# zgcr/SimpleAICV_pytorch_training_examples

Hardware: AMD Instinct MI355X
Metric: training images/sec/node (higher is better)
Workload: dtype bf16; 1 GPU; resnet50 3x224x224 synthetic training step (fwd+loss+bwd+all-reduce+optimizer), per-GPU batch 256; model=resnet50, global_batch=256, per_gpu_batch=256, parallelism=dp1, step_graph=True, bn_statistics=fixed-order partial rows, deterministic=True, loop=tools.scripts.train_classification, optimizer=SGD, param_groups=2

## Files before the change

simpleaicv_pytorch_training_examples_amd/csrc/igemm.hip:

```cpp
#include <type_traits>

#include <stdlib.h>
#include "common.h"
#include "saicv_internal.h"
#include "det.h"
#include "../../include/saicv_hip.h"

namespace {

struct FastDiv {
    uint32_t mul, s1, s2;
};
DEVINL uint32_t fdiv(uint32_t n, FastDiv d) {
    const uint32_t t = __umulhi(d.mul, n);
    return (t + ((n - t) >> d.s1)) >> d.s2;
}

constexpr int nt_stages(int bm, int bn) { return (bm == 256 && bn == 128) ? 3 : 4; }
constexpr int nt_stages_kc8(int bm, int bn) { return (bm + bn) * 128 * 3 <= 150 * 1024 ? 3 : 2; }

struct NTParams {
    const void* src;
    const void* wgt;
    void* out;
// ... 752 lines not shown
    if (bstats) {
        __syncthreads();
        float* red = reinterpret_cast<float*>(smem);
        const bool have = ncol + OEPC <= p.Nn;
#pragma unroll
        for (int j = 0; j < OEPC; ++j) {
            const float mu = have ? p.bs_mean[ncol + j] : 0.f, is = have ? p.bs_invstd[ncol + j] : 0.f;
            red[(orow0 * 2 + 0) * BN_T + oc * OEPC + j] = bag[j];
            red[(orow0 * 2 + 1) * BN_T + oc * OEPC + j] = is * fmaf(-mu, bag[j], bax[j]);
        }
        __syncthreads();
        const size_t prow = (size_t)((MODE == 1 && cs > 1) ? blockIdx.y : 0) * p.bs_rows + tile_m;
        for (int c = tid; c < 2 * BN_T; c += NTHREADS) {
            const int which = c / BN_T, col = c - which * BN_T;
            float a = 0.f;
            for (int r = 0; r < RPP; ++r) a += red[(r * 2 + which) * BN_T + col];
            const int n = tile_n * BN_T + col;
            if (n < p.Nn) {
                float* dst = (which ? p.bs_gx : p.bs_g) + (p.stat_atomic_rows ? prow % p.stat_atomic_rows : prow) * (size_t)p.Nn + n;
                if (p.stat_atomic_rows) unsafeAtomicAdd(dst, a); else *dst = a;
            }
        }
    }
    }
#ifdef SAICV_NT_TIMELINE
    if (tl_on && tix == (int)blockIdx.x) {
        NT_STAMP(6);
        asm volatile("s_waitcnt vmcnt(0)" ::: "memory");
        NT_STAMP(7);
        if (tid == 0) {
            unsigned long long* rec = p.timeline + ((size_t)blockIdx.y * gridDim.x + blockIdx.x) * 16;
            unsigned int hw, xcc;
            asm volatile("s_getreg_b32 %0, hwreg(HW_REG_HW_ID)" : "=s"(hw));
            asm volatile("s_getreg_b32 %0, hwreg(HW_REG_XCC_ID)" : "=s"(xcc));
#pragma unroll
            for (int i = 0; i < 8; ++i) rec[i] = tl_t[i];
            rec[8] = ((unsigned long long)xcc << 32) | hw;
            rec[9] = __builtin_amdgcn_s_memrealtime();
            rec[10] = tl_rt0;
            rec[11] = tl_t[8]; rec[12] = tl_t[9]; rec[13] = tl_t[10];
        }
    }
#endif
    }
}


struct TNParams {
    const void* dy;
    const void* src;
    float* dw;
    float* dbias;
    uint32_t dy_bytes, src_bytes;
    int H, W, C;
    int OH, OW;
    int R, S, stride, pad;
    int M, Cout, Kd;
    int tiles_a, tiles_b;
    int m_per_split;
    int d_img, d_oh, d_ow;
    FastDiv fd_ohw, fd_ow;
    saicv::DetSink det;
};

template <typename T, int BA, int BB, int NWA, int NWB>
__global__ __launch_bounds__(64 * NWA * NWB) void igemm_tn_kernel(const TNParams p) {
    constexpr int THREADS = 64 * NWA * NWB;
    constexpr int EPC = ElemTraits<T>::EPC;
    constexpr int BR = 8 * EPC;
    constexpr int PITCH_A = (BA + 16) * (int)sizeof(T);
    constexpr int PITCH_B = (BB + 16) * (int)sizeof(T);
    constexpr int A_BYTES = BR * PITCH_A;
    constexpr int B_BYTES = BR * PITCH_B;
    constexpr int STAGE = A_BYTES + B_BYTES;
    constexpr int CPR_A = BA / EPC, CPR_B = BB / EPC;
    constexpr int RPP_A = THREADS / CPR_A, RPP_B = THREADS / CPR_B;
    constexpr int NA = BR / RPP_A, NB = BR / RPP_B;
    constexpr int WA = BA / NWA, WB = BB / NWB;
    constexpr int AT = WA / 16, BT = WB / 16;
    constexpr uint32_t OOB = 0xfffffff0u;

    extern __shared__ __attribute__((aligned(16))) char smem[];
    const int tid = threadIdx.x;
    const int lane = tid & 63;
    const int wave = tid >> 6;
    const int wa = wave % NWA, wb = wave / NWA;
    const int l15 = lane & 15, lg = lane >> 4;

    const int ntile = gridDim.x;
    const int lid = xcd_remap(blockIdx.y * ntile + blockIdx.x, ntile * gridDim.y);
    const int split = lid / ntile;
    const int tile = lid - split * ntile;
    const int tile_a = tile % p.tiles_a;
    const int tile_b = tile / p.tiles_a;
    const int m_begin = split * p.m_per_split;
    const int m_end = min(p.M, m_begin + p.m_per_split);
    if (m_begin >= m_end) return;

    const __amdgpu_buffer_rsrc_t dy_rs =
        __builtin_amdgcn_make_buffer_rsrc(const_cast<void*>(p.dy), 0, p.dy_bytes, 0x00020000);
    const __amdgpu_buffer_rsrc_t src_rs =
        __builtin_amdgcn_make_buffer_rsrc(const_cast<void*>(p.src), 0, p.src_bytes, 0x00020000);

    const int ca = tid % CPR_A, rba = tid / CPR_A;
    const int n_ld = tile_a * BA + ca * EPC;
    const bool n_ok = n_ld < p.Cout;
    uint32_t dy_off = (uint32_t)((m_begin + rba) * p.Cout + n_ld) * (uint32_t)sizeof(T);
    const uint32_t dy_row_step = (uint32_t)(RPP_A * p.Cout) * (uint32_t)sizeof(T);
    const uint32_t dy_tile_step = (uint32_t)(BR * p.Cout) * (uint32_t)sizeof(T);
    int m_a = m_begin + rba;
    const int cb = tid % CPR_B, rbb = tid / CPR_B;
    const int kk_ld = tile_b * BB + cb * EPC;
    const bool kk_ok = kk_ld < p.Kd;
    const int tap = kk_ld / p.C;
    const int c0 = kk_ld - tap * p.C;
    const int fr = tap / p.S - p.pad;
    const int fs = tap - (tap / p.S) * p.S - p.pad;
    int g_img[NB], g_oh[NB], g_ow[NB];
    const int ohw = p.OH * p.OW;
#pragma unroll
    for (int i = 0; i < NB; ++i) {
        const int m = m_begin + rbb + RPP_B * i;
        const int img = (int)fdiv((uint32_t)m, p.fd_ohw);
        const int rem = m - img * ohw;
        g_img[i] = img;
        g_oh[i] = (int)fdiv((uint32_t)rem, p.fd_ow);
        g_ow[i] = rem - g_oh[i] * p.OW;
    }
    int m_b = m_begin + rbb;

    u32x4 ra[NA], rbv[NB];
    const bool do_bias = (p.dbias != nullptr) && (tile_b == 0);
    float bsum[EPC];
#pragma unroll
    for (int k = 0; k < EPC; ++k) bsum[k] = 0.f;
    auto load_tile = [&]() {
#pragma unroll
        for (int i = 0; i < NA; ++i) {
            const bool ok = n_ok & (m_a + RPP_A * i < m_end);
            ra[i] = buf_ld(dy_rs, ok ? dy_off + (uint32_t)i * dy_row_step : OOB);
        }
        dy_off += dy_tile_step;
        m_a += BR;
#pragma unroll
        for (int i = 0; i < NB; ++i) {
            const int ih = g_oh[i] * p.stride + fr;
            const int iw = g_ow[i] * p.stride + fs;
            const bool ok = kk_ok & (m_b + RPP_B * i < m_end) & ((unsigned)ih < (unsigned)p.H) &
                            ((unsigned)iw < (unsigned)p.W);
            const uint32_t off = (uint32_t)(((g_img[i] * p.H + ih) * p.W + iw) * p.C + c0) * (uint32_t)sizeof(T);
            rbv[i] = buf_ld(src_rs, ok ? off : OOB);
            int ow = g_ow[i] + p.d_ow;
            int cy = ow >= p.OW;
            ow -= cy ? p.OW : 0;
            int oh = g_oh[i] + p.d_oh + cy;
            cy = oh >= p.OH;
            oh -= cy ? p.OH : 0;
            g_ow[i] = ow;
            g_oh[i] = oh;
            g_img[i] += p.d_img + cy;
        }
        m_b += BR;
    };
    int st_a[NA], st_b[NB];
#pragma unroll
    for (int i = 0; i < NA; ++i) st_a[i] = (rba + RPP_A * i) * PITCH_A + ca * 16;
#pragma unroll
    for (int i = 0; i < NB; ++i) st_b[i] = A_BYTES + (rbb + RPP_B * i) * PITCH_B + cb * 16;
    auto store_tile = [&](int stage) {
        char* base = smem + stage * STAGE;
        if (do_bias) {
#pragma unroll
            for (int i = 0; i < NA; ++i) {
                float f[EPC];
                Chunk<T>::unpack(ra[i], f);
#pragma unroll
                for (int k = 0; k < EPC; ++k) bsum[k] += f[k];
            }
        }
#pragma unroll
        for (int i = 0; i < NA; ++i) st_chunk(base + st_a[i], ra[i]);
#pragma unroll
        for (int i = 0; i < NB; ++i) st_chunk(base + st_b[i], rbv[i]);
    };

    f32x4 acc[AT][BT];
#pragma unroll
    for (int ai = 0; ai < AT; ++ai)
#pragma unroll
        for (int bi = 0; bi < BT; ++bi) acc[ai][bi] = f32x4{0.f, 0.f, 0.f, 0.f};

    int fa_off[AT], fb_off[BT];
    if constexpr (sizeof(T) == 2) {
        const int row0 = lg * 8 + (l15 >> 2);
#pragma unroll
        for (int ai = 0; ai < AT; ++ai) fa_off[ai] = row0 * PITCH_A + (wa * WA + ai * 16 + (l15 & 3) * 4) * 2;
#pragma unroll
        for (int bi = 0; bi < BT; ++bi) fb_off[bi] = A_BYTES + row0 * PITCH_B + (wb * WB + bi * 16 + (l15 & 3) * 4) * 2;
    } else {
#pragma unroll
        for (int ai = 0; ai < AT; ++ai) fa_off[ai] = lg * PITCH_A + (wa * WA + ai * 16 + l15) * 4;
#pragma unroll
        for (int bi = 0; bi < BT; ++bi) fb_off[bi] = A_BYTES + lg * PITCH_B + (wb * WB + bi * 16 + l15) * 4;
    }

    auto compute = [&](int stage) {
        const char* base = smem + stage * STAGE;
        if constexpr (sizeof(T) == 2) {
            typedef __attribute__((address_space(3))) bf16x4 lds_bf16x4;
#pragma unroll
            for (int ks = 0; ks < 2; ++ks) {
                u32x4 af[AT], bf[BT];
#pragma unroll
                for (int ai = 0; ai < AT; ++ai) {
                    const char* q = base + fa_off[ai] + ks * 32 * PITCH_A;
                    bf16x4 lo = __builtin_amdgcn_ds_read_tr16_b64_v4bf16((lds_bf16x4*)(q));
                    bf16x4 hi = __builtin_amdgcn_ds_read_tr16_b64_v4bf16((lds_bf16x4*)(q + 4 * PITCH_A));
                    u32x2 l2 = __builtin_bit_cast(u32x2, lo), h2 = __builtin_bit_cast(u32x2, hi);
                    af[ai] = u32x4{l2[0], l2[1], h2[0], h2[1]};
                }
#pragma unroll
                for (int bi = 0; bi < BT; ++bi) {
                    const char* q = base + fb_off[bi] + ks * 32 * PITCH_B;
                    bf16x4 lo = __builtin_amdgcn_ds_read_tr16_b64_v4bf16((lds_bf16x4*)(q));
                    bf16x4 hi = __builtin_amdgcn_ds_read_tr16_b64_v4bf16((lds_bf16x4*)(q + 4 * PITCH_B));
                    u32x2 l2 = __builtin_bit_cast(u32x2, lo), h2 = __builtin_bit_cast(u32x2, hi);
                    bf[bi] = u32x4{l2[0], l2[1], h2[0], h2[1]};
                }
#pragma unroll
                for (int ai = 0; ai < AT; ++ai)
#pragma unroll
                    for (int bi = 0; bi < BT; ++bi)
                        acc[ai][bi] = __builtin_amdgcn_mfma_f32_16x16x32_bf16(
                            __builtin_bit_cast(bf16x8, af[ai]), __builtin_bit_cast(bf16x8, bf[bi]),
                            acc[ai][bi], 0, 0, 0);
            }
        } else {
#pragma unroll
            for (int ks = 0; ks < BR / 4; ++ks) {
                float af[AT], bf[BT];
#pragma unroll
                for (int ai = 0; ai < AT; ++ai)
                    af[ai] = *reinterpret_cast<const float*>(base + fa_off[ai] + ks * 4 * PITCH_A);
#pragma unroll
                for (int bi = 0; bi < BT; ++bi)
                    bf[bi] = *reinterpret_cast<const float*>(base + fb_off[bi] + ks * 4 * PITCH_B);
#pragma unroll
                for (int ai = 0; ai < AT; ++ai)
#pragma unroll
                    for (int bi = 0; bi < BT; ++bi)
                        acc[ai][bi] = __builtin_amdgcn_mfma_f32_16x16x4f32(af[ai], bf[bi],
                                                                          acc[ai][bi], 0, 0, 0);
            }
        }
    };

    const int nt = (m_end - m_begin + BR - 1) / BR;
    load_tile();
    store_tile(0);
    __syncthreads();
    for (int t = 0; t < nt; ++t) {
        const int cur = t & 1;
        const bool more = (t + 1) < nt;
        if (more) load_tile();
        compute(cur);
        if (more) store_tile(cur ^ 1);
        __syncthreads();
    }

    if (do_bias) {
        float* red = reinterpret_cast<float*>(smem);
#pragma unroll
        for (int k = 0; k < EPC; ++k) red[tid * EPC + k] = bsum[k];
        __syncthreads();
        if (rba == 0 && n_ok) {
#pragma unroll
            for (int k = 0; k < EPC; ++k) {
                float sgm = 0.f;
                for (int t = 0; t < RPP_A; ++t) sgm += red[(t * CPR_A + ca) * EPC + k];
                saicv::det_add(p.det, p.dbias + n_ld + k, (size_t)p.Cout * p.Kd + n_ld + k, split, sgm);
            }
        }
    }
#pragma unroll
    for (int ai = 0; ai < AT; ++ai) {
        const int n0 = tile_a * BA + wa * WA + ai * 16 + lg * 4;
#pragma unroll
        for (int bi = 0; bi < BT; ++bi) {
            const int kk = tile_b * BB + wb * WB + bi * 16 + l15;
            if (kk < p.Kd) {
#pragma unroll
                for (int r = 0; r < 4; ++r)
                    if (n0 + r < p.Cout)
                        saicv::det_add(p.det, p.dw + (size_t)(n0 + r) * (size_t)p.Kd + kk, (size_t)(n0 + r) * (size_t)p.Kd + kk, split, acc[ai][bi][r]);
            }
        }
    }
}

DEVINL int tn_key(int r) { return (r & 3) | (((r >> 3) & 1) << 2); }
template <int CPR> DEVINL int tn_g(int r) { return CPR >= 16 ? tn_key(r) : (tn_key(r) >> 1); }

template <int BA, int BB, int NWA, int NWB, bool PLAIN>
__global__ __launch_bounds__(64 * NWA * NWB) void igemm_tn_dma_kernel(const TNParams p) {
    typedef bf16_t T;
    constexpr int NWAVES = NWA * NWB;
    constexpr int BR = 32;
    constexpr int CPR_A = BA / 8, CPR_B = BB / 8;
    constexpr int RPI_A = 64 / CPR_A, RPI_B = 64 / CPR_B;
    constexpr int NIA = (BR / RPI_A) / NWAVES, NIB = (BR / RPI_B) / NWAVES;
    static_assert(NIA >= 1 && NIB >= 1 && NIA * NWAVES * RPI_A == BR && NIB * NWAVES * RPI_B == BR, "tile / wavefront split");
    constexpr int LPT = NIA + NIB;
    constexpr int PITCH_A = BA * 2, PITCH_B = BB * 2;
    constexpr int A_BYTES = BR * PITCH_A, B_BYTES = BR * PITCH_B;
    constexpr int STAGE = A_BYTES + B_BYTES;
    constexpr int NSTAGE = 4;
    constexpr int WA = BA / NWA, WB = BB / NWB;
    constexpr int AT = WA / 16, BT = WB / 16;
    static_assert(AT % NWB == 0, "bias-gradient tiles per wavefront");
    constexpr int ABT = AT / NWB;
    constexpr uint32_t OOB = 0xfffffff0u;

    extern __shared__ __attribute__((aligned(16))) char smem[];
    const int tid = threadIdx.x;
    const int lane = tid & 63;
    const int wave = __builtin_amdgcn_readfirstlane(tid >> 6);
    const int wa = wave % NWA, wb = wave / NWA;
    const int l15 = lane & 15, lg = lane >> 4;

    const int ntile = gridDim.x;
    const int lid = xcd_remap(blockIdx.y * ntile + blockIdx.x, ntile * gridDim.y);
    const int split = lid / ntile;
    const int tile = lid - split * ntile;
    const int tile_a = tile % p.tiles_a;
    const int tile_b = tile / p.tiles_a;
    const int m_begin = split * p.m_per_split;
    const int m_end = min(p.M, m_begin + p.m_per_split);
    if (m_begin >= m_end) return;

    const __amdgpu_buffer_rsrc_t dy_rs =
        __builtin_amdgcn_make_buffer_rsrc(const_cast<void*>(p.dy), 0, p.dy_bytes, 0x00020000);
    const __amdgpu_buffer_rsrc_t src_rs =
        __builtin_amdgcn_make_buffer_rsrc(const_cast<void*>(p.src), 0, p.src_bytes, 0x00020000);

    uint32_t a_off[NIA];
    int a_m[NIA];
    bool a_ok[NIA];
#pragma unroll
    for (int i = 0; i < NIA; ++i) {
        const int row = (i * NWAVES + wave) * RPI_A + lane / CPR_A;
        const int chunk = (lane % CPR_A) ^ (tn_g<CPR_A>(row) << 1);
        const int n = tile_a * BA + chunk * 8;
        a_ok[i] = n < p.Cout;
        a_m[i] = m_begin + row;
        a_off[i] = (uint32_t)((m_begin + row) * p.Cout + n) * 2u;
    }
    const uint32_t a_step = (uint32_t)(BR * p.Cout) * 2u;
    uint32_t b_off[NIB];
    int b_m[NIB], g_oh[NIB], g_ow[NIB], b_fr[NIB], b_fs[NIB];
    bool b_ok[NIB];
    const int ohw = p.OH * p.OW;
    const int st_dow = p.stride * p.d_ow, st_ow = p.stride * p.OW, st_doh = p.stride * p.d_oh, st_oh = p.stride * p.OH;
    const uint32_t inc_base = (uint32_t)(((p.d_img * p.H + st_doh) * p.W + st_dow) * p.C) * 2u;
    const uint32_t inc_cy1 = (uint32_t)((p.stride * p.W - st_ow) * p.C) * 2u;
    const uint32_t inc_cy2 = (uint32_t)(((p.H - st_oh) * p.W) * p.C) * 2u;
#pragma unroll
    for (int j = 0; j < NIB; ++j) {
        const int row = (j * NWAVES + wave) * RPI_B + lane / CPR_B;
        const int chunk = (lane % CPR_B) ^ (tn_g<CPR_B>(row) << 1);
        const int kk = tile_b * BB + chunk * 8;
        b_ok[j] = kk < p.Kd;
        const int m = m_begin + row;
        b_m[j] = m;
        if (PLAIN) {
            b_off[j] = (uint32_t)(m * p.C + kk) * 2u;
            g_oh[j] = g_ow[j] = b_fr[j] = b_fs[j] = 0;
        } else {
            const int tap = kk / p.C;
            const int c0 = kk - tap * p.C;
            b_fr[j] = tap / p.S - p.pad;
            b_fs[j] = tap - (tap / p.S) * p.S - p.pad;
            const int img = (int)fdiv((uint32_t)m, p.fd_ohw);
            const int rem = m - img * ohw;
            g_oh[j] = (int)fdiv((uint32_t)rem, p.fd_ow);
            g_ow[j] = rem - g_oh[j] * p.OW;
            const int ih0 = g_oh[j] * p.stride + b_fr[j], iw0 = g_ow[j] * p.stride + b_fs[j];
            b_off[j] = (uint32_t)(((img * p.H + ih0) * p.W + iw0) * p.C + c0) * 2u;
        }
    }
    const uint32_t b_step = (uint32_t)(BR * p.C) * 2u;

    typedef __attribute__((address_space(3))) void lds_void;
    auto issue_step = [&](int stage) __attribute__((always_inline)) {
        char* base = smem + stage * STAGE + wave * 1024;
#pragma unroll
        for (int i = 0; i < NIA; ++i) {
            const bool ok = a_ok[i] & (a_m[i] < m_end);
            __builtin_amdgcn_raw_ptr_buffer_load_lds(dy_rs, (lds_void*)(base + i * NWAVES * 1024), 16, (int)(ok ? a_off[i] : OOB), 0, 0, 0);
            a_off[i] += a_step;
            a_m[i] += BR;
        }
#pragma unroll
        for (int j = 0; j < NIB; ++j) {
            if (PLAIN) {
                const bool ok = b_ok[j] & (b_m[j] < m_end);
                __builtin_amdgcn_raw_ptr_buffer_load_lds(src_rs, (lds_void*)(base + A_BYTES + j * NWAVES * 1024), 16, (int)(ok ? b_off[j] : OOB), 0, 0, 0);
                b_off[j] += b_step;
            } else {
                const int ih = __mul24(g_oh[j], p.stride) + b_fr[j];
                const int iw = __mul24(g_ow[j], p.stride) + b_fs[j];
                const bool ok = b_ok[j] & (b_m[j] < m_end) & ((unsigned)ih < (unsigned)p.H) & ((unsigned)iw < (unsigned)p.W);
                __builtin_amdgcn_raw_ptr_buffer_load_lds(src_rs, (lds_void*)(base + A_BYTES + j * NWAVES * 1024), 16, (int)(ok ? b_off[j] : OOB), 0, 0, 0);
                int ow = g_ow[j] + p.d_ow;
                const bool c1 = ow >= p.OW;
                ow -= c1 ? p.OW : 0;
                int oh = g_oh[j] + p.d_oh + (c1 ? 1 : 0);
                const bool c2 = oh >= p.OH;
                oh -= c2 ? p.OH : 0;
                g_ow[j] = ow;
                g_oh[j] = oh;
                b_off[j] += inc_base + (c1 ? inc_cy1 : 0u) + (c2 ? inc_cy2 : 0u);
            }
            b_m[j] += BR;
        }
    };

    f32x4 acc[AT][BT];
#pragma unroll
    for (int ai = 0; ai < AT; ++ai)
#pragma unroll
        for (int bi = 0; bi < BT; ++bi) acc[ai][bi] = f32x4{0.f, 0.f, 0.f, 0.f};
    const bool do_bias = (p.dbias != nullptr) && (tile_b == 0);
    f32x4 bacc[ABT];
#pragma unroll
    for (int t = 0; t < ABT; ++t) bacc[t] = f32x4{0.f, 0.f, 0.f, 0.f};

    const int row0 = lg * 8 + (l15 >> 2);
    int fa_off[AT], fb_off[BT];
#pragma unroll
    for (int ai = 0; ai < AT; ++ai)
        fa_off[ai] = row0 * PITCH_A + (((wa * AT + ai) ^ tn_g<CPR_A>(row0)) << 5) + (l15 & 3) * 8;
#pragma unroll
    for (int bi = 0; bi < BT; ++bi)
        fb_off[bi] = A_BYTES + row0 * PITCH_B + (((wb * BT + bi) ^ tn_g<CPR_B>(row0)) << 5) + (l15 & 3) * 8;

    const u32x4 ones = {0x3F803F80u, 0x3F803F80u, 0x3F803F80u, 0x3F803F80u};
    auto compute = [&](int stage) __attribute__((always_inline)) {
        const uint32_t base = (uint32_t)(uintptr_t)(__attribute__((address_space(3))) char*)(smem + stage * STAGE);
        u32x2 alo[AT], ahi[AT], blo[BT], bhi[BT];
#pragma unroll
        for (int ai = 0; ai < AT; ++ai) {
            const uint32_t q = base + (uint32_t)fa_off[ai];
            asm volatile("ds_read_b64_tr_b16 %0, %2\n\tds_read_b64_tr_b16 %1, %2 offset:%3"
                         : "=&v"(alo[ai]), "=&v"(ahi[ai]) : "v"(q), "n"(4 * PITCH_A) : "memory");
        }
#pragma unroll
        for (int bi = 0; bi < BT; ++bi) {
            const uint32_t q = base + (uint32_t)fb_off[bi];
            asm volatile("ds_read_b64_tr_b16 %0, %2\n\tds_read_b64_tr_b16 %1, %2 offset:%3"
                         : "=&v"(blo[bi]), "=&v"(bhi[bi]) : "v"(q), "n"(4 * PITCH_B) : "memory");
        }
        u32x4 af[AT];
#pragma unroll
        for (int bi = 0; bi < BT; ++bi) {
            asm volatile("s_waitcnt lgkmcnt(%2)" : "+v"(blo[bi]), "+v"(bhi[bi]) : "n"(2 * (BT - 1 - bi)) : "memory");
            if (bi == 0) {
#pragma unroll
                for (int ai = 0; ai < AT; ++ai) af[ai] = u32x4{alo[ai][0], alo[ai][1], ahi[ai][0], ahi[ai][1]};
            }
            const u32x4 bf = {blo[bi][0], blo[bi][1], bhi[bi][0], bhi[bi][1]};
#pragma unroll
            for (int ai = 0; ai < AT; ++ai)
                acc[ai][bi] = __builtin_amdgcn_mfma_f32_16x16x32_bf16(__builtin_bit_cast(bf16x8, af[ai]),
                                                                      __builtin_bit_cast(bf16x8, bf), acc[ai][bi], 0, 0, 0);
        }
        if (do_bias) {
#pragma unroll
            for (int t = 0; t < ABT; ++t)
                bacc[t] = __builtin_amdgcn_mfma_f32_16x16x32_bf16(__builtin_bit_cast(bf16x8, af[wb * ABT + t]),
                                                                  __builtin_bit_cast(bf16x8, ones), bacc[t], 0, 0, 0);
        }
    };

    const int nt = (m_end - m_begin + BR - 1) / BR;
    int issued = 0;
    for (; issued < NSTAGE - 1 && issued < nt; ++issued) issue_step(issued);
    int st_c = 0;
    int st_i = issued % NSTAGE;
    for (int t = 0; t < nt; ++t) {
        const int ahead = issued - t - 1;
        if (ahead >= 2) asm volatile("s_waitcnt vmcnt(%0)" ::"n"(2 * LPT) : "memory");
        else if (ahead == 1) asm volatile("s_waitcnt vmcnt(%0)" ::"n"(LPT) : "memory");
        else asm volatile("s_waitcnt vmcnt(0)" ::: "memory");
        __builtin_amdgcn_s_barrier();
        if (issued < nt) {
            issue_step(st_i);
            ++issued;
            st_i = (st_i + 1 == NSTAGE) ? 0 : st_i + 1;
        }
        compute(st_c);
        st_c = (st_c + 1 == NSTAGE) ? 0 : st_c + 1;
    }

    if (do_bias && l15 == 0) {
#pragma unroll
        for (int t = 0; t < ABT; ++t) {
            const int n0 = tile_a * BA + wa * WA + (wb * ABT + t) * 16 + lg * 4;
#pragma unroll
            for (int r = 0; r < 4; ++r)
                if (n0 + r < p.Cout) saicv::det_add(p.det, p.dbias + n0 + r, (size_t)p.Cout * p.Kd + n0 + r, split, bacc[t][r]);
        }
    }
#pragma unroll
    for (int ai = 0; ai < AT; ++ai) {
        const int n0 = tile_a * BA + wa * WA + ai * 16 + lg * 4;
#pragma unroll
        for (int bi = 0; bi < BT; ++bi) {
            const int kk = tile_b * BB + wb * WB + bi * 16 + l15;
            if (kk < p.Kd) {
#pragma unroll
                for (int r = 0; r < 4; ++r)
                    if (n0 + r < p.Cout)
                        saicv::det_add(p.det, p.dw + (size_t)(n0 + r) * (size_t)p.Kd + kk, (size_t)(n0 + r) * (size_t)p.Kd + kk, split, acc[ai][bi][r]);
            }
        }
    }
}

FastDiv make_fastdiv(uint32_t d) {
    FastDiv f;
    uint32_t l = 0;
    while ((1ull << l) < d) ++l;
    f.mul = (uint32_t)(((1ull << 32) * ((1ull << l) - d)) / d + 1);
    f.s1 = l < 1 ? l : 1;
    f.s2 = l > 0 ? l - 1 : 0;
    return f;
}

template <typename K>
void allow_lds(K k, size_t smem) {
    hipFuncSetAttribute(reinterpret_cast<const void*>(k), hipFuncAttributeMaxDynamicSharedMemorySize, (int)smem);
}

template <typename T, int BM_T, int BN_T, int WM_, int WN_, int MODE, bool OUT_F32, bool PLAIN, int KC = 4>
int launch_nt1_inst(const NTParams& p, size_t smem, hipStream_t st) {
    auto k = igemm_nt1_kernel<T, BM_T, BN_T, WM_, WN_, MODE, OUT_F32, PLAIN, KC>;
    static bool once = (allow_lds(k, 160 * 1024), true);
    (void)once;
    dim3 grid(p.nblk, (MODE == 1 && p.stride > 1) ? p.stride * p.stride : 1), block(64 * WM_ * WN_);
    hipLaunchKernelGGL(k, grid, block, smem, st, p);
    return saicv::check_launch("igemm_nt");
}

template <typename T, int BM_T, int BN_T, int WM_, int WN_, int MODE>
int launch_nt1(const NTParams& p, bool out_f32, bool plain, hipStream_t st) {
    constexpr bool F32_OUT = !(BM_T == 256 && BN_T == 256) && (sizeof(T) == 4 || MODE == 0);
    constexpr bool BF16_OUT = sizeof(T) == 2;
    constexpr size_t smem_full = nt_stages(BM_T, BN_T) * (size_t)(BM_T * 64 + BN_T * 64);
    const size_t epi = BM_T * (size_t)(BN_T * ((out_f32 || sizeof(T) == 4) ? 4 : 2) + 16) +
                       2 * WM_ * BN_T * sizeof(float);
    size_t smem = smem_full;
    if (smem < epi) smem = epi;
#ifdef SAICV_NT_TIMELINE
    if (getenv("SAICV_NT_SOLO") && smem < 84 * 1024) smem = 84 * 1024;
#endif
    if constexpr (BF16_OUT && BM_T == 256) {
        if (p.kc8 && plain && !out_f32) {
            constexpr size_t ring = nt_stages_kc8(BM_T, BN_T) * (size_t)(BM_T + BN_T) * 128;
            return launch_nt1_inst<T, BM_T, BN_T, WM_, WN_, MODE, false, true, 8>(p, ring < epi ? epi : ring, st);
        }
    }
    if constexpr (F32_OUT) {
        if (out_f32) {
            if (plain) return launch_nt1_inst<T, BM_T, BN_T, WM_, WN_, MODE, true, true>(p, smem, st);
            return launch_nt1_inst<T, BM_T, BN_T, WM_, WN_, MODE, true, false>(p, smem, st);
        }
    }
    if constexpr (BF16_OUT) {
        if (!out_f32) {
            if (plain) return launch_nt1_inst<T, BM_T, BN_T, WM_, WN_, MODE, false, true>(p, smem, st);
            return launch_nt1_inst<T, BM_T, BN_T, WM_, WN_, MODE, false, false>(p, smem, st);
        }
    }
    saicv::set_error("igemm_nt: the %d x %d tile has no %s-output form for %s data", BM_T, BN_T, out_f32 ? "fp32" : "bf16",
                     sizeof(T) == 2 ? "bf16" : "fp32");
    return -1;
}

struct NTTile { int bm, bn, blocks_per_cu; float speed; };
const NTTile kTiles[4] = {{256, 256, 1, 0.80f}, {256, 128, 2, 1.00f}, {128, 128, 2, 0.60f}, {128, 64, 3, 0.50f}};

int pick_tile(int M, int Nn, int nkt, bool f32_out_big) {
    if (const char* force = getenv("SAICV_NT_TILE")) {
        const int t = atoi(force);
        if (t >= 0 && t < 4 && !(f32_out_big && kTiles[t].bm * kTiles[t].bn * 4 > 150 * 1024)) return t;
    }
    int best = 2;
    float best_score = -1.f;
    for (int t = 0; t < 4; ++t) {
        if (f32_out_big && kTiles[t].bm * kTiles[t].bn * 4 > 150 * 1024) continue;
        const NTTile& g = kTiles[t];
        const long tm = (M + g.bm - 1) / g.bm, tn = (Nn + g.bn - 1) / g.bn;
        const float blocks = (float)(tm * tn);
        const float slots = 256.f * g.blocks_per_cu;
        const float rounds = blocks / slots;
        const float quant = rounds / (float)(long)(rounds + 0.999999f);
        const float useful = ((float)M / (tm * g.bm)) * ((float)Nn / (tn * g.bn));
        float speed = g.speed;
        if (t == 0) speed = nkt >= 100 ? 1.10f : nkt >= 48 ? 0.90f : 0.80f;
        const float score = speed * quant * useful;
        if (score > best_score) { best_score = score; best = t; }
    }
    return best;
}

struct NTProblem {
    int dtype, mode;
    int H, W, C, OH, OW, R, S, stride, pad;
    int M, Nn, Kd, ldo;
    bool out_f32;
    bool bias, stats, addend, row_scale, out2, bn_sums;
    int act_mode;
};
enum NTRoute { NT_TILED, NT_PW_STREAM, NT_PW3_STREAM };
struct NTPlan {
    NTRoute route;
    int tile;
    bool kc8;
    bool plain;
    bool f32o;
    int blocks;
    int stat_rows;
};

NTPlan nt_plan(const NTProblem& q) {
    NTPlan pl = {NT_TILED, 0, false, false, false, 0, 0};
    const bool streamable = q.dtype == SAICV_DTYPE_BF16 && !q.out_f32 && q.stride == 1 && q.ldo == q.Nn && !q.bias && !q.act_mode &&
                            !q.row_scale && !q.out2 && !(q.stats && (q.addend || q.bn_sums));
    if (streamable && q.R == 1 && q.S == 1 && q.pad == 0) {
        pl.blocks = saicv::pw_stream_blocks(q.dtype, q.M, q.Nn, q.Kd, (q.addend || q.bn_sums) && !q.stats);
        if (pl.blocks > 0) {
            pl.route = NT_PW_STREAM;
            pl.stat_rows = pl.blocks;
            return pl;
        }
    }
    if (streamable && q.R == 3 && q.S == 3 && q.pad == 1 && q.C == 64 && q.H == q.OH && q.W == q.OW && q.H >= 1 && q.W >= 1 &&
        q.M % (q.H * q.W) == 0) {
        pl.blocks = saicv::pw3_stream_blocks(q.dtype, q.M, q.Nn, q.Kd);
        if (pl.blocks > 0) {
            pl.route = NT_PW3_STREAM;
            pl.stat_rows = pl.blocks;
            return pl;
        }
    }
    const bool f32o = q.out_f32 || q.dtype == SAICV_DTYPE_F32;
    int M_tile = q.M;
    if (q.mode == 1 && q.stride > 1)
        M_tile = (q.M / (q.OH * q.OW)) * ((q.OH + q.stride - 1) / q.stride) * ((q.OW + q.stride - 1) / q.stride);
    const int bk = q.dtype == SAICV_DTYPE_BF16 ? 32 : 16;
    pl.tile = pick_tile(M_tile, q.Nn, (q.Kd + bk - 1) / bk, f32o);
    const char* ke = getenv("SAICV_NT_KC8");
    const int kc8_mode = ke ? atoi(ke) : 2;
    const bool pointwise = q.R == 1 && q.S == 1 && q.pad == 0 && (q.mode == 0 || q.stride == 1);
    pl.plain = pointwise;
    pl.f32o = f32o;
    const bool ok = q.dtype == SAICV_DTYPE_BF16 && !f32o && pointwise && kTiles[pl.tile].bm == 256 && q.Kd >= 256;
    if (ok && kc8_mode == 1) pl.kc8 = true;
    const bool rule_ok = (kc8_mode == 2 && q.act_mode == 0) || kc8_mode == 3;
    if (ok && rule_ok && q.Nn >= 2048 && q.Nn % 256 == 0 && q.Kd >= 512 && (long)((M_tile + 255) / 256) * (q.Nn / 256) >= 4 * 256) {
        pl.kc8 = true;
        pl.tile = 0;
    }
    const int classes = q.mode == 1 && q.stride > 1 ? q.stride * q.stride : 1;
    pl.stat_rows = ((M_tile + kTiles[pl.tile].bm - 1) / kTiles[pl.tile].bm) * classes;
    pl.blocks = pl.stat_rows * ((q.Nn + kTiles[pl.tile].bn - 1) / kTiles[pl.tile].bn);
    return pl;
}

bool nt_operands_fit(const NTProblem& q) {
    const size_t esz = q.dtype == SAICV_DTYPE_BF16 ? 2 : 4;
    const size_t src_bytes = (size_t)(q.M / (q.OH * q.OW)) * q.H * q.W * q.C * esz;
    const size_t wgt_bytes = (size_t)q.Nn * q.Kd * esz;
    return src_bytes < 0xfffffff0ull && wgt_bytes < 0xfffffff0ull;
}

struct TNProblem {
    int dtype;
    int H, W, C, OH, OW, R, S, stride, pad;
    int M, Cout, Kd;
};
struct TNPlan {
    bool big;
    int ba, bb;
    int tiles_a, tiles_b;
    int BR;
    int total_rt;
    int rt_per;
    int splits;
    bool dma;
    bool plain;
};

TNPlan tn_plan(const TNProblem& q) {
    TNPlan pl;
    const int epc = q.dtype == SAICV_DTYPE_BF16 ? 8 : 4;
    const int M = q.M, Cout = q.Cout, Kd = q.Kd;
    const int BR = 8 * epc;
    pl.BR = BR;
    static const int force_big = getenv("SAICV_TN_BIG") ? atoi(getenv("SAICV_TN_BIG")) : -1;
    const int big_tiles = ((Cout + 255) / 256) * ((Kd + 255) / 256);
    const int big_steps = ((M + BR - 1) / BR) / (256 / big_tiles > 0 ? 256 / big_tiles : 1);
    const bool big = force_big >= 0 ? (force_big != 0 && Cout >= 128 && Kd >= 128)
                                    : (Cout % 256 == 0 && Kd >= 256 && (Kd % 256 == 0 || Kd >= 1024) && big_steps >= 48);
    pl.big = big;
    const int ba = big ? 256 : Cout <= 64 ? 64 : 128;
    const int bb = big ? 256 : Kd <= 64 ? 64 : 128;
    pl.ba = ba; pl.bb = bb;
    pl.tiles_a = (Cout + ba - 1) / ba;
    pl.tiles_b = (Kd + bb - 1) / bb;
    const int tiles = pl.tiles_a * pl.tiles_b;
    const int total_rt = (M + BR - 1) / BR;
    const char* slots_env = getenv("SAICV_TN_SLOTS_PCT");
    const int slots_pct = slots_env ? atoi(slots_env) : (g_saicv_comm_world > 1 ? 85 : 100);
    int splits = ((big ? 256 : 512) * slots_pct / 100) / tiles;
    if (splits > total_rt) splits = total_rt;
    if (splits < 1) splits = 1;
    int rt_per = (total_rt + splits - 1) / splits;
    splits = (total_rt + rt_per - 1) / rt_per;
    pl.total_rt = total_rt; pl.rt_per = rt_per; pl.splits = splits;
    const char* de = getenv("SAICV_TN_DMA");
    const int use_dma = de ? atoi(de) : 1;
    pl.dma = use_dma && q.dtype == SAICV_DTYPE_BF16;
    pl.plain = q.R == 1 && q.S == 1 && q.stride == 1 && q.pad == 0 && q.H == q.OH && q.W == q.OW;
    return pl;
}

bool tn_operands_fit(const TNProblem& q) {
    const size_t esz = q.dtype == SAICV_DTYPE_BF16 ? 2 : 4;
    const size_t dy_bytes = (size_t)q.M * q.Cout * esz;
    const size_t src_bytes = (size_t)(q.M / (q.OH * q.OW)) * q.H * q.W * q.C * esz;
    return dy_bytes < 0xfffffff0ull && src_bytes < 0xfffffff0ull;
}

template <typename T, int BA, int BB, int NWA = 2, int NWB = 2>
int launch_tn(const TNParams& p, int splits, hipStream_t st) {
    constexpr int EPC = ElemTraits<T>::EPC;
    constexpr int BR = 8 * EPC;
    constexpr size_t smem = 2 * (size_t)BR * ((BA + 16) + (BB + 16)) * sizeof(T);
    dim3 grid(p.tiles_a * p.tiles_b, splits), block(64 * NWA * NWB);
    auto k = igemm_tn_kernel<T, BA, BB, NWA, NWB>;
    static bool once = (allow_lds(k, smem), true);
    (void)once;
    hipLaunchKernelGGL(k, grid, block, smem, st, p);
    return saicv::check_launch("igemm_tn");
}

template <int BA, int BB, int NWA = 2, int NWB = 2>
int launch_tn_dma(const TNParams& p, int splits, bool plain, hipStream_t st) {
    constexpr size_t smem = 4 * (size_t)32 * (BA + BB) * 2;
    dim3 grid(p.tiles_a * p.tiles_b, splits), block(64 * NWA * NWB);
    if (plain) {
        auto k = igemm_tn_dma_kernel<BA, BB, NWA, NWB, true>;
        static bool once = (allow_lds(k, smem), true);
        (void)once;
        hipLaunchKernelGGL(k, grid, block, smem, st, p);
    } else {
        auto k = igemm_tn_dma_kernel<BA, BB, NWA, NWB, false>;
        static bool once = (allow_lds(k, smem), true);
        (void)once;
        hipLaunchKernelGGL(k, grid, block, smem, st, p);
    }
    return saicv::check_launch("igemm_tn");
}

}

namespace saicv {

int conv_stat_rows(const saicv_conv_desc* d) {
    const NTProblem q = {d->dtype, 0, d->H, d->W, d->C, d->OH, d->OW, d->R, d->S, d->stride, d->pad,
                         d->N * d->OH * d->OW, d->K, d->R * d->S * d->C, d->K,
                         false, false, true, false, false, false, false, 0};
    return nt_plan(q).stat_rows;
}

int conv_bwd_stat_rows(const saicv_conv_desc* d) {
    const NTProblem q = {d->dtype, 1, d->OH, d->OW, d->K, d->H, d->W, d->R, d->S, d->stride, d->pad,
                         d->N * d->H * d->W, d->C, d->R * d->S * d->K, d->C,
                         false, false, false, false, false, false, true, 0};
    return nt_plan(q).stat_rows;
}

int igemm_nt(int dtype, int mode, const void* src, const void* wgt, void* out, const float* bias,
             float* stat_sum, float* stat_sq, int H, int W, int C, int OH, int OW, int R, int S,
             int stride, int pad, int M, int Nn, int Kd, int ldo, int out_f32, hipStream_t st,
             const EpiExtra* ex) {
    const int epc = dtype == SAICV_DTYPE_BF16 ? 8 : 4;
    SAICV_REQUIRE(C % epc == 0, "igemm_nt: C=%d must be a multiple of %d", C, epc);
    SAICV_REQUIRE(Kd % epc == 0, "igemm_nt: Kd=%d must be a multiple of %d", Kd, epc);
    SAICV_REQUIRE(M > 0 && Nn > 0 && Kd > 0, "igemm_nt: empty problem");
    SAICV_REQUIRE(!(bias && stat_sum), "igemm_nt: bias and BN statistics are exclusive");
    NTParams p;
    p.src = src; p.wgt = wgt; p.out = out; p.bias = bias; p.stat_sum = stat_sum; p.stat_sq = stat_sq;
    p.addend = ex ? ex->addend : nullptr;
    p.row_scale = ex ? ex->row_scale : nullptr;
    p.rows_per_scale = ex ? ex->rows_per_scale : 1;
    p.out2 = ex ? ex->out2 : nullptr;
    p.act_mode = ex ? ex->act_mode : 0;
    static const int lean_gelu_env = getenv("SAICV_GELU_EPI") ? atoi(getenv("SAICV_GELU_EPI")) : 1;
    p.lean_gelu = lean_gelu_env;
    p.addend_gate = ex ? ex->addend_gate : nullptr;
    p.bs_y = ex ? ex->bs_y : nullptr;
    p.bs_mask = ex ? ex->bs_mask : nullptr;
    p.bs_mean = ex ? ex->bs_mean : nullptr;
    p.bs_invstd = ex ? ex->bs_invstd : nullptr;
    p.bs_g = ex ? ex->bs_g : nullptr;
    p.bs_gx = ex ? ex->bs_gx : nullptr;
    p.bs_rows = 0;
    p.stat_atomic_rows = ex ? ex->stat_atomic_rows : 0;
#ifdef SAICV_NT_TIMELINE
// ... 203 lines not shown
```

Measured before the change: 12630 images/s.

## Software-pipeline LDS fragment reads in weight-gradient DMA GEMM kernel

Restructures the weight-gradient (TN) implicit-GEMM kernel so the next stage's LDS fragments are read while the current stage's MFMAs run. Small tiles use double-buffered register fragment sets; large tiles interleave per-tile refills between MFMA rows. The prologue always issues all stages, leaning on out-of-bounds buffer loads returning zero. Per-iteration register arrays (row counters, ok flags, filter offsets) collapse into scalars, tile offsets become XOR masks, and launch bounds request two blocks per CU for 4-wave configs. These aim to hide LDS latency and cut register pressure, at the cost of more live fragment registers and possible spills.

```diff
diff --git a/simpleaicv_pytorch_training_examples_amd/csrc/igemm.hip b/simpleaicv_pytorch_training_examples_amd/csrc/igemm.hip
--- a/simpleaicv_pytorch_training_examples_amd/csrc/igemm.hip
+++ b/simpleaicv_pytorch_training_examples_amd/csrc/igemm.hip
@@ -1078,7 +1078,7 @@
 template <int CPR> DEVINL int tn_g(int r) { return CPR >= 16 ? tn_key(r) : (tn_key(r) >> 1); }
 
 template <int BA, int BB, int NWA, int NWB, bool PLAIN>
-__global__ __launch_bounds__(64 * NWA * NWB) void igemm_tn_dma_kernel(const TNParams p) {
+__global__ __launch_bounds__(64 * NWA * NWB, NWA * NWB == 4 ? 2 : 1) void igemm_tn_dma_kernel(const TNParams p) {
     typedef bf16_t T;
     constexpr int NWAVES = NWA * NWB;
     constexpr int BR = 32;
@@ -1119,22 +1119,22 @@
     const __amdgpu_buffer_rsrc_t src_rs =
         __builtin_amdgcn_make_buffer_rsrc(const_cast<void*>(p.src), 0, p.src_bytes, 0x00020000);
 
+    static_assert((NWAVES * RPI_A) % 16 == 0 && (NWAVES * RPI_B) % 16 == 0, "one column chunk per thread");
     uint32_t a_off[NIA];
-    int a_m[NIA];
-    bool a_ok[NIA];
-#pragma unroll
-    for (int i = 0; i < NIA; ++i) {
-        const int row = (i * NWAVES + wave) * RPI_A + lane / CPR_A;
-        const int chunk = (lane % CPR_A) ^ (tn_g<CPR_A>(row) << 1);
+    int a_m = m_begin + wave * RPI_A + lane / CPR_A;
+    bool a_ok;
+    {
+        const int chunk = (lane % CPR_A) ^ (tn_g<CPR_A>(wave * RPI_A + lane / CPR_A) << 1);
         const int n = tile_a * BA + chunk * 8;
-        a_ok[i] = n < p.Cout;
-        a_m[i] = m_begin + row;
-        a_off[i] = (uint32_t)((m_begin + row) * p.Cout + n) * 2u;
+        a_ok = n < p.Cout;
+#pragma unroll
+        for (int i = 0; i < NIA; ++i) a_off[i] = (uint32_t)((a_m + i * NWAVES * RPI_A) * p.Cout + n) * 2u;
     }
     const uint32_t a_step = (uint32_t)(BR * p.Cout) * 2u;
     uint32_t b_off[NIB];
-    int b_m[NIB], g_oh[NIB], g_ow[NIB], b_fr[NIB], b_fs[NIB];
-    bool b_ok[NIB];
+    int b_m = m_begin + wave * RPI_B + lane / CPR_B;
+    int g_oh[NIB], g_ow[NIB], b_fr = 0, b_fs = 0;
+    bool b_ok;
     const int ohw = p.OH * p.OW;
     const int st_dow = p.stride * p.d_ow, st_ow = p.stride * p.OW, st_doh = p.stride * p.d_oh, st_oh = p.stride * p.OH;
     const uint32_t inc_base = (uint32_t)(((p.d_img * p.H + st_doh) * p.W + st_dow) * p.C) * 2u;
@@ -1145,22 +1145,21 @@
         const int row = (j * NWAVES + wave) * RPI_B + lane / CPR_B;
         const int chunk = (lane % CPR_B) ^ (tn_g<CPR_B>(row) << 1);
         const int kk = tile_b * BB + chunk * 8;
-        b_ok[j] = kk < p.Kd;
+        b_ok = kk < p.Kd;
         const int m = m_begin + row;
-        b_m[j] = m;
         if (PLAIN) {
             b_off[j] = (uint32_t)(m * p.C + kk) * 2u;
-            g_oh[j] = g_ow[j] = b_fr[j] = b_fs[j] = 0;
+            g_oh[j] = g_ow[j] = 0;
         } else {
             const int tap = kk / p.C;
             const int c0 = kk - tap * p.C;
-            b_fr[j] = tap / p.S - p.pad;
-            b_fs[j] = tap - (tap / p.S) * p.S - p.pad;
+            b_fr = tap / p.S - p.pad;
+            b_fs = tap - (tap / p.S) * p.S - p.pad;
             const int img = (int)fdiv((uint32_t)m, p.fd_ohw);
             const int rem = m - img * ohw;
             g_oh[j] = (int)fdiv((uint32_t)rem, p.fd_ow);
             g_ow[j] = rem - g_oh[j] * p.OW;
-            const int ih0 = g_oh[j] * p.stride + b_fr[j], iw0 = g_ow[j] * p.stride + b_fs[j];
+            const int ih0 = g_oh[j] * p.stride + b_fr, iw0 = g_ow[j] * p.stride + b_fs;
             b_off[j] = (uint32_t)(((img * p.H + ih0) * p.W + iw0) * p.C + c0) * 2u;
         }
     }
@@ -1171,21 +1170,21 @@
         char* base = smem + stage * STAGE + wave * 1024;
 #pragma unroll
         for (int i = 0; i < NIA; ++i) {
-            const bool ok = a_ok[i] & (a_m[i] < m_end);
+            const bool ok = a_ok & (a_m < m_end - i * NWAVES * RPI_A);
             __builtin_amdgcn_raw_ptr_buffer_load_lds(dy_rs, (lds_void*)(base + i * NWAVES * 1024), 16, (int)(ok ? a_off[i] : OOB), 0, 0, 0);
             a_off[i] += a_step;
-            a_m[i] += BR;
-        }
+        }
+        a_m += BR;
 #pragma unroll
         for (int j = 0; j < NIB; ++j) {
             if (PLAIN) {
-                const bool ok = b_ok[j] & (b_m[j] < m_end);
+                const bool ok = b_ok & (b_m < m_end - j * NWAVES * RPI_B);
                 __builtin_amdgcn_raw_ptr_buffer_load_lds(src_rs, (lds_void*)(base + A_BYTES + j * NWAVES * 1024), 16, (int)(ok ? b_off[j] : OOB), 0, 0, 0);
                 b_off[j] += b_step;
             } else {
-                const int ih = __mul24(g_oh[j], p.stride) + b_fr[j];
-                const int iw = __mul24(g_ow[j], p.stride) + b_fs[j];
-                const bool ok = b_ok[j] & (b_m[j] < m_end) & ((unsigned)ih < (unsigned)p.H) & ((unsigned)iw < (unsigned)p.W);
+                const int ih = __mul24(g_oh[j], p.stride) + b_fr;
+                const int iw = __mul24(g_ow[j], p.stride) + b_fs;
+                const bool ok = b_ok & (b_m < m_end - j * NWAVES * RPI_B) & ((unsigned)ih < (unsigned)p.H) & ((unsigned)iw < (unsigned)p.W);
                 __builtin_amdgcn_raw_ptr_buffer_load_lds(src_rs, (lds_void*)(base + A_BYTES + j * NWAVES * 1024), 16, (int)(ok ? b_off[j] : OOB), 0, 0, 0);
                 int ow = g_ow[j] + p.d_ow;
                 const bool c1 = ow >= p.OW;
@@ -1197,8 +1196,8 @@
                 g_oh[j] = oh;
                 b_off[j] += inc_base + (c1 ? inc_cy1 : 0u) + (c2 ? inc_cy2 : 0u);
             }
-            b_m[j] += BR;
-        }
+        }
+        b_m += BR;
     };
 
     f32x4 acc[AT][BT];
@@ -1212,76 +1211,145 @@
     for (int t = 0; t < ABT; ++t) bacc[t] = f32x4{0.f, 0.f, 0.f, 0.f};
 
     const int row0 = lg * 8 + (l15 >> 2);
-    int fa_off[AT], fb_off[BT];
-#pragma unroll
-    for (int ai = 0; ai < AT; ++ai)
-        fa_off[ai] = row0 * PITCH_A + (((wa * AT + ai) ^ tn_g<CPR_A>(row0)) << 5) + (l15 & 3) * 8;
-#pragma unroll
-    for (int bi = 0; bi < BT; ++bi)
-        fb_off[bi] = A_BYTES + row0 * PITCH_B + (((wb * BT + bi) ^ tn_g<CPR_B>(row0)) << 5) + (l15 & 3) * 8;
+    uint32_t fa_off0 = row0 * PITCH_A + (((wa * AT) ^ tn_g<CPR_A>(row0)) << 5) + (l15 & 3) * 8;
+    uint32_t fb_off0 = A_BYTES + row0 * PITCH_B + (((wb * BT) ^ tn_g<CPR_B>(row0)) << 5) + (l15 & 3) * 8;
+    static_assert((AT & (AT - 1)) == 0 && (BT & (BT - 1)) == 0 && (A_BYTES & (PITCH_B - 1)) == 0, "tile offsets as XOR masks");
 
     const u32x4 ones = {0x3F803F80u, 0x3F803F80u, 0x3F803F80u, 0x3F803F80u};
-    auto compute = [&](int stage) __attribute__((always_inline)) {
+    constexpr bool TWO_SETS = AT * BT <= 16;
+    struct FragA {
+        u32x2 lo[AT], hi[AT];
+    };
+    struct FragB {
+        u32x2 lo[BT], hi[BT];
+    };
+    FragA fa0, fa1;
+    FragB fb0, fb1;
+    auto read_a_tile = [&](FragA& f, int ai, int stage) __attribute__((always_inline)) {
         const uint32_t base = (uint32_t)(uintptr_t)(__attribute__((address_space(3))) char*)(smem + stage * STAGE);
-        u32x2 alo[AT], ahi[AT], blo[BT], bhi[BT];
+        const uint32_t q = base + (fa_off0 ^ (uint32_t)(ai << 5));
+        asm volatile("ds_read_b64_tr_b16 %0, %2\n\tds_read_b64_tr_b16 %1, %2 offset:%3"
+                     : "=&v"(f.lo[ai]), "=&v"(f.hi[ai]) : "v"(q), "n"(4 * PITCH_A) : "memory");
+    };
+    auto read_a = [&](FragA& f, int stage) __attribute__((always_inline)) {
+#pragma unroll
+        for (int ai = 0; ai < AT; ++ai) read_a_tile(f, ai, stage);
+    };
+    auto read_b_tile = [&](FragB& f, int bi, int stage) __attribute__((always_inline)) {
+        const uint32_t base = (uint32_t)(uintptr_t)(__attribute__((address_space(3))) char*)(smem + stage * STAGE);
+        const uint32_t q = base + (fb_off0 ^ (uint32_t)(bi << 5));
+        asm volatile("ds_read_b64_tr_b16 %0, %2\n\tds_read_b64_tr_b16 %1, %2 offset:%3"
+                     : "=&v"(f.lo[bi]), "=&v"(f.hi[bi]) : "v"(q), "n"(4 * PITCH_B) : "memory");
+    };
+    auto read_b = [&](FragB& f, int stage) __attribute__((always_inline)) {
+#pragma unroll
+        for (int bi = 0; bi < BT; ++bi) read_b_tile(f, bi, stage);
+    };
+    auto release_frags = [&](FragA& a, FragB& b) __attribute__((always_inline)) {
+        __builtin_amdgcn_sched_barrier(0);
+#define TN_FA(i) "+v"(a.lo[i]), "+v"(a.hi[i])
+#define TN_FB(i) "+v"(b.lo[i]), "+v"(b.hi[i])
+        if constexpr (AT == 2 && BT == 2) asm volatile("s_waitcnt lgkmcnt(0)" : TN_FA(0), TN_FA(1), TN_FB(0), TN_FB(1)::"memory");
+        if constexpr (AT == 2 && BT == 4)
+            asm volatile("s_waitcnt lgkmcnt(0)" : TN_FA(0), TN_FA(1), TN_FB(0), TN_FB(1), TN_FB(2), TN_FB(3)::"memory");
+        if constexpr (AT == 4 && BT == 2)
+            asm volatile("s_waitcnt lgkmcnt(0)" : TN_FA(0), TN_FA(1), TN_FA(2), TN_FA(3), TN_FB(0), TN_FB(1)::"memory");
+        if constexpr (AT == 4 && BT == 4)
+            asm volatile("s_waitcnt lgkmcnt(0)" : TN_FA(0), TN_FA(1), TN_FA(2), TN_FA(3), TN_FB(0), TN_FB(1), TN_FB(2), TN_FB(3)::"memory");
+        if constexpr (AT == 8 && BT == 4)
+            asm volatile("s_waitcnt lgkmcnt(0)"
+                         : TN_FA(0), TN_FA(1), TN_FA(2), TN_FA(3), TN_FA(4), TN_FA(5), TN_FA(6), TN_FA(7), TN_FB(0), TN_FB(1), TN_FB(2), TN_FB(3)::"memory");
+        static_assert((AT == 2 && BT == 2) || (AT == 2 && BT == 4) || (AT == 4 && BT == 2) || (AT == 4 && BT == 4) || (AT == 8 && BT == 4),
+                      "no release statement for this tile");
+#undef TN_FA
+#undef TN_FB
+    };
+    auto mma_step = [&](FragA& a, FragB& b, auto bias_tag, auto refill_tag, int next_slot) __attribute__((always_inline)) {
+        constexpr bool BIAS = decltype(bias_tag)::value, REFILL = decltype(refill_tag)::value;
+        u32x4 af[AT], bf[BT];
+#pragma unroll
+        for (int ai = 0; ai < AT; ++ai) af[ai] = u32x4{a.lo[ai][0], a.lo[ai][1], a.hi[ai][0], a.hi[ai][1]};
+#pragma unroll
+        for (int bi = 0; bi < BT; ++bi) bf[bi] = u32x4{b.lo[bi][0], b.lo[bi][1], b.hi[bi][0], b.hi[bi][1]};
+        if constexpr (BIAS) {
+#pragma unroll
+            for (int t = 0; t < ABT; ++t) {
+                u32x4 ab = af[t];
+#pragma unroll
+                for (int w = 1; w < NWB; ++w) ab = (wb == w) ? af[w * ABT + t] : ab;
+                bacc[t] = __builtin_amdgcn_mfma_f32_16x16x32_bf16(__builtin_bit_cast(bf16x8, ab),
+                                                                  __builtin_bit_cast(bf16x8, ones), bacc[t], 0, 0, 0);
+            }
+        }
 #pragma unroll
         for (int ai = 0; ai < AT; ++ai) {
-            const uint32_t q = base + (uint32_t)fa_off[ai];
-            asm volatile("ds_read_b64_tr_b16 %0, %2\n\tds_read_b64_tr_b16 %1, %2 offset:%3"
-                         : "=&v"(alo[ai]), "=&v"(ahi[ai]) : "v"(q), "n"(4 * PITCH_A) : "memory");
-        }
-#pragma unroll
-        for (int bi = 0; bi < BT; ++bi) {
-            const uint32_t q = base + (uint32_t)fb_off[bi];
-            asm volatile("ds_read_b64_tr_b16 %0, %2\n\tds_read_b64_tr_b16 %1, %2 offset:%3"
-                         : "=&v"(blo[bi]), "=&v"(bhi[bi]) : "v"(q), "n"(4 * PITCH_B) : "memory");
-        }
-        u32x4 af[AT];
-#pragma unroll
-        for (int bi = 0; bi < BT; ++bi) {
-            asm volatile("s_waitcnt lgkmcnt(%2)" : "+v"(blo[bi]), "+v"(bhi[bi]) : "n"(2 * (BT - 1 - bi)) : "memory");
-            if (bi == 0) {
-#pragma unroll
-                for (int ai = 0; ai < AT; ++ai) af[ai] = u32x4{alo[ai][0], alo[ai][1], ahi[ai][0], ahi[ai][1]};
-            }
-            const u32x4 bf = {blo[bi][0], blo[bi][1], bhi[bi][0], bhi[bi][1]};
-#pragma unroll
-            for (int ai = 0; ai < AT; ++ai)
+#pragma unroll
+            for (int bi = 0; bi < BT; ++bi)
                 acc[ai][bi] = __builtin_amdgcn_mfma_f32_16x16x32_bf16(__builtin_bit_cast(bf16x8, af[ai]),
-                                                                      __builtin_bit_cast(bf16x8, bf), acc[ai][bi], 0, 0, 0);
-        }
-        if (do_bias) {
-#pragma unroll
-            for (int t = 0; t < ABT; ++t)
-                bacc[t] = __builtin_amdgcn_mfma_f32_16x16x32_bf16(__builtin_bit_cast(bf16x8, af[wb * ABT + t]),
-                                                                  __builtin_bit_cast(bf16x8, ones), bacc[t], 0, 0, 0);
+                                                                      __builtin_bit_cast(bf16x8, bf[bi]), acc[ai][bi], 0, 0, 0);
+            if constexpr (REFILL) {
+                __builtin_amdgcn_sched_barrier(0);
+                read_a_tile(a, ai, next_slot);
+            }
+        }
+        if constexpr (REFILL) {
+            read_b(b, next_slot);
+            release_frags(a, b);
         }
     };
 
     const int nt = (m_end - m_begin + BR - 1) / BR;
-    int issued = 0;
-    for (; issued < NSTAGE - 1 && issued < nt; ++issued) issue_step(issued);
-    int st_c = 0;
-    int st_i = issued % NSTAGE;
-    for (int t = 0; t < nt; ++t) {
-        const int ahead = issued - t - 1;
-        if (ahead >= 2) asm volatile("s_waitcnt vmcnt(%0)" ::"n"(2 * LPT) : "memory");
-        else if (ahead == 1) asm volatile("s_waitcnt vmcnt(%0)" ::"n"(LPT) : "memory");
-        else asm volatile("s_waitcnt vmcnt(0)" ::: "memory");
+    static_assert((NSTAGE & (NSTAGE - 1)) == 0, "ring slots by mask");
+#pragma unroll
+    for (int s = 0; s < NSTAGE; ++s) issue_step(s);
+#pragma unroll
+    for (int i = 0; i < NIA; ++i) asm volatile("" : "+v"(a_off[i]));
+#pragma unroll
+    for (int j = 0; j < NIB; ++j) asm volatile("" : "+v"(b_off[j]));
+    asm volatile("" : "+v"(a_m), "+v"(b_m));
+    asm volatile("s_waitcnt vmcnt(%0)" ::"n"((NSTAGE - 1) * LPT) : "memory");
+    __builtin_amdgcn_s_barrier();
+    read_a(fa0, 0);
+    read_b(fb0, 0);
+    release_frags(fa0, fb0);
+
+    auto k_step = [&](FragA& cura, FragB& curb, FragA& nxta, FragB& nxtb, int slot, auto bias_tag) __attribute__((always_inline)) {
+        asm volatile("s_waitcnt vmcnt(%0) ; tn_dma steady state" ::"n"((NSTAGE - 2) * LPT) : "memory");
         __builtin_amdgcn_s_barrier();
-        if (issued < nt) {
-            issue_step(st_i);
-            ++issued;
-            st_i = (st_i + 1 == NSTAGE) ? 0 : st_i + 1;
-        }
-        compute(st_c);
-        st_c = (st_c + 1 == NSTAGE) ? 0 : st_c + 1;
-    }
-
-    if (do_bias && l15 == 0) {
+        asm volatile("" : "+v"(fa_off0), "+v"(fb_off0));
+        issue_step(slot);
+        const int next_slot = (slot + 1) & (NSTAGE - 1);
+        if constexpr (TWO_SETS) {
+            read_a(nxta, next_slot);
+            read_b(nxtb, next_slot);
+            mma_step(cura, curb, bias_tag, std::false_type{}, 0);
+            release_frags(nxta, nxtb);
+        } else {
+            mma_step(cura, curb, bias_tag, std::true_type{}, next_slot);
+        }
+    };
+    auto k_loop = [&](auto bias_tag) __attribute__((always_inline)) {
+        if constexpr (TWO_SETS) {
+            const int n_pairs = nt & ~1;
+            for (int t = 0; t < n_pairs; t += 2) {
+                k_step(fa0, fb0, fa1, fb1, t & (NSTAGE - 1), bias_tag);
+                k_step(fa1, fb1, fa0, fb0, (t + 1) & (NSTAGE - 1), bias_tag);
+            }
+            if (nt & 1) k_step(fa0, fb0, fa1, fb1, n_pairs & (NSTAGE - 1), bias_tag);
+        } else {
+            for (int t = 0; t < nt; ++t) k_step(fa0, fb0, fa1, fb1, t & (NSTAGE - 1), bias_tag);
+        }
+    };
+    if (do_bias) k_loop(std::true_type{});
+    else k_loop(std::false_type{});
+    asm volatile("s_waitcnt vmcnt(0)" ::: "memory");
+    const int lane_e = __builtin_amdgcn_mbcnt_hi(~0u, __builtin_amdgcn_mbcnt_lo(~0u, 0u));
+    const int l15e = lane_e & 15, lge = lane_e >> 4;
+
+    if (do_bias && l15e == 0) {
 #pragma unroll
         for (int t = 0; t < ABT; ++t) {
-            const int n0 = tile_a * BA + wa * WA + (wb * ABT + t) * 16 + lg * 4;
+            const int n0 = tile_a * BA + wa * WA + (wb * ABT + t) * 16 + lge * 4;
 #pragma unroll
             for (int r = 0; r < 4; ++r)
                 if (n0 + r < p.Cout) saicv::det_add(p.det, p.dbias + n0 + r, (size_t)p.Cout * p.Kd + n0 + r, split, bacc[t][r]);
@@ -1289,10 +1357,10 @@
     }
 #pragma unroll
     for (int ai = 0; ai < AT; ++ai) {
-        const int n0 = tile_a * BA + wa * WA + ai * 16 + lg * 4;
+        const int n0 = tile_a * BA + wa * WA + ai * 16 + lge * 4;
 #pragma unroll
         for (int bi = 0; bi < BT; ++bi) {
-            const int kk = tile_b * BB + wb * WB + bi * 16 + l15;
+            const int kk = tile_b * BB + wb * WB + bi * 16 + l15e;
             if (kk < p.Kd) {
 #pragma unroll
                 for (int r = 0; r < 4; ++r)
```

Measured after the change: 12740 images/s, median of 6. About the same (+0.9%).
